# fenghansen/YOND_public

Hardware: AMD Instinct MI355X
Metric: Bayer megapixels/sec end-to-end (NLE+VST+denoise+iVST) (higher is better)
Workload: dtype f32 (3x3 convolutions: f32 operands as two f16 halves -- 22-23 significant bits -- on the f16 MFMA, 3 products per f32 product, f32 accumulate; per-layer error vs float64 asserted <= 2x the f32 direct kernel's and <= 2e-5 of max|ref| (tests/test_hip_conv.py; measured 1.3e-6 vs 1.5e-6), whole frame v

## Files before the change

### include/yond_hip.h

```cpp
#ifndef YOND_HIP_H
#define YOND_HIP_H

#include <stddef.h>
#include <stdint.h>

#ifdef __cplusplus
extern "C" {
#endif

#define YOND_OK 0
#define YOND_EINVAL (-1)
#define YOND_EUNSUPPORTED (-2)

#define YOND_ABI_VERSION 8
int yond_abi_version(void);

int yond_pack_vst_norm_f32(const float* bayer, int H, int W, float* out, int pad_l, int pad_r, int pad_t,
                           int pad_b, int mode, double scale, double gain, double sigma, double lo,
                           double hi, const double* lut_x, const float* lut_y, int lut_n, float* img_max,
                           void* stream);

int yond_pack_vst_norm_biaslut_f32(const float* bayer, int H, int W, float* out, int pad_l, int pad_r, int pad_t,
                                   int pad_b, double scale, double gain, double sigma, double lo, double hi,
                                   const double* lut_x, const double* lut_y, int lut_n, float* img_max, void* stream);
// ... 27 lines not shown

typedef struct YondConvDesc {
    const float* src0;
    const float* src1;
    int C0, C1;
    int N, H, W;
    int Ho, Wo;
    int Cout;
    int ksize;
    int stride;
    int shuffle;
    int pre_act;
    int post_act;
    float slope;
    const float* wpk;
    const float* escale;
    const float* eshift;
    int ebatch;
    const float* res;
    float* dst;
    int tn;
    int kc;
    int algo;
    const float* out4_w;
    const float* out4_b;
    const float* out4_x;
    const float* out4_ub;
    float* out4_dst;
    unsigned int* status;
    int in_fmt, out_fmt;
    int res_fmt;
    unsigned long long* clk;
    int tile_order;
    float* dst2;
} YondConvDesc;
#define YOND_STATUS_HALF_OVERFLOW 1u
#define YOND_FMT_NHWC_F32 0
#define YOND_FMT_SPLIT_PLANES 1
#define YOND_FMT_PLANES4 2
#define YOND_SP_PLANE_UNITS(H, W) ((((H) * (W)) + 8) / 8 * 8)
#define YOND_SP_BYTES(N, C, H, W) ((size_t)(N) * ((C) / 16) * 4 * (size_t)YOND_SP_PLANE_UNITS(H, W) * 16)
#define YOND_HP_BYTES(N, C, H, W) ((size_t)(N) * ((C) / 16) * 2 * (size_t)YOND_SP_PLANE_UNITS(H, W) * 16)

int yond_conv_config(int ksize, int stride, int cin, int cout, int shuffle, int N, int Ho, int Wo, int* tn, int* kc);
int yond_pack_conv_weight_f32(const float* w, int cout, int cin, int ksize, int tn, int kc, float* dst);
int yond_pack_conv_weight_split_f32(const float* w, int cout, int cin, int ksize, int tn, int kc, float* dst);
int yond_conv2d_f32(const YondConvDesc* desc, void* stream);

int yond_conv_wino_supported(int cin, int cout);
int yond_pack_conv_wino_weight_f32(const float* w, int cout, int cin, int tn, float* dst);

int yond_conv_split_supported(int ksize, int stride, int cin, int cout);
int yond_pack_conv_split_weight_f32(const float* w, int cout, int cin, int ksize, int tn, int parts, float* dst);
int yond_pack_conv_split_weight_dev_f32(const float* w, int cout, int cin, int ksize, int tn, int parts, float* dst, int* status,
                                        void* stream);
int yond_pack_conv_split_weights_batch_dev_f32(const float* src, const long long* desc, int nlayers, float* dst, size_t ngroups,
                                               int* status, void* stream);

int yond_conv_in_f32(const float* x, const float* ub , int N, int H, int W, int Cout,
                     const float* wpk, const float* bias, float slope, float* dst,
                     int out_fmt , void* stream);
int yond_pack_conv_in_weight_f32(const float* w , int cout, float* dst );

int yond_conv_out_f32(const float* feat , int Cin, const float* w ,
                      const float* bias , const float* x ,
                      const float* ub , int N, int H, int W, float* dst ,
                      void* stream);

int yond_maxpool2_f32(const float* src, int N, int H, int W, int C, float* dst, void* stream);

typedef struct YondFilmDesc {
    int kind, C, ld;
    const float *w_a0, *b_a0, *w_a2, *b_a2;
    const float *w_b0, *b_b0;
    const float *w_b, *b_b;
    const float *cb1, *cb2;
    float *s1, *t1, *s2, *t2;
} YondFilmDesc;
int yond_film_f32(const YondFilmDesc* descs, int nblocks, const float* t , const float* ub ,
                  int N, void* stream);

int yond_box_stats_self1_f32(const float* bayer, int H, int W, int k, int k2, int tile_w, float* mean,
                             float* var, float* blur2, void* stream);
int yond_box_stats_self2_f32(const float* blur2, int h, int w, int k, int tile_w, float* lap, void* stream);
int yond_box_stats_collab_f32(const float* bayer_lr, const float* bayer_hr, int H, int W, int k, int tile_w,
                              float* mean, float* var, float* lap, void* stream);


int yond_box_stats_self_stats_f32(const float* bayer, int H, int W, int k, int k2, int tile_w, float* mean, float* var,
                                  float* blur2, float* lap, const double* q_host, int nq, void* ws, void* stream);
int yond_box_stats_collab_stats_f32(const float* bayer_lr, const float* bayer_hr, int H, int W, int k, int tile_w,
                                    float* mean, float* var, float* lap, const double* q_host, int nq, void* ws, void* stream);

size_t yond_select_ws_bytes(int nr);
int yond_select_ranks_f32(const float* data, size_t n, const int64_t* ranks_host, int nr, float* out, void* ws,
                          void* stream);
int yond_percentiles_f32(const float* data, size_t n, const double* q_host, int nq, double* out, void* ws,
                         void* stream);

size_t yond_nle_ws_bytes(size_t n);
int yond_nle_stats_f32(const float* lap, const float* mean, size_t n, int width, const double* q_host, int nq, void* ws,
                       void* stream);
int yond_nle_threshold_f32(const float* lap, size_t n, const double* q_host, int nq, int want_score, void* ws, void* stream);
int yond_nle_state_layout(int* off );
int yond_nle_moments_f32(const float* lap, const float* mean, const float* var, size_t n, void* ws, void* stream);

// ... 214 lines not shown
```

### yond_public_amd/_lib.py

```python
import ctypes as C
import os

import torch

_HERE = os.path.dirname(os.path.abspath(__file__))
LIB_PATH = os.environ.get("YOND_HIP_LIB", os.path.join(_HERE, "libyond_hip.so"))
_lib = None
ABI_VERSION = 8

vp, i32, f32, f64, sz, i64 = C.c_void_p, C.c_int, C.c_float, C.c_double, C.c_size_t, C.c_longlong


class YondConvDesc(C.Structure):
    _fields_ = [("src0", vp), ("src1", vp), ("C0", i32), ("C1", i32), ("N", i32), ("H", i32), ("W", i32),
                ("Ho", i32), ("Wo", i32), ("Cout", i32), ("ksize", i32), ("stride", i32), ("shuffle", i32),
                ("pre_act", i32), ("post_act", i32), ("slope", f32), ("wpk", vp), ("escale", vp),
                ("eshift", vp), ("ebatch", i32), ("res", vp), ("dst", vp), ("tn", i32), ("kc", i32), ("algo", i32),
                ("out4_w", vp), ("out4_b", vp), ("out4_x", vp), ("out4_ub", vp), ("out4_dst", vp), ("status", vp),
                ("in_fmt", i32), ("out_fmt", i32), ("res_fmt", i32), ("clk", vp), ("tile_order", i32), ("dst2", vp)]


class YondBlock0Desc(C.Structure):
    _fields_ = [("x", vp), ("in_fmt", i32), ("N", i32), ("H", i32), ("W", i32), ("w1", vp), ("w2", vp),
                ("s1", vp), ("t1", vp), ("s2", vp), ("t2", vp), ("ebatch", i32), ("dst", vp),
                ("out4_w", vp), ("out4_b", vp), ("out4_x", vp), ("out4_ub", vp), ("out4_dst", vp), ("status", vp)]


class YondFilmDesc(C.Structure):
    _fields_ = [("kind", i32), ("C", i32), ("ld", i32),
                ("w_a0", vp), ("b_a0", vp), ("w_a2", vp), ("b_a2", vp), ("w_b0", vp), ("b_b0", vp),
                ("w_b", vp), ("b_b", vp), ("cb1", vp), ("cb2", vp),
                ("s1", vp), ("t1", vp), ("s2", vp), ("t2", vp)]


PROTOTYPES = {
    "yond_abi_version": [],
    "yond_pack_vst_norm_f32": [vp, i32, i32, vp, i32, i32, i32, i32, i32, f64, f64, f64, f64, f64, vp, vp, i32, vp, vp],
    "yond_pack_vst_norm_biaslut_f32": [vp, i32, i32, vp, i32, i32, i32, i32, f64, f64, f64, f64, f64, vp, vp, i32, vp, vp],
    "yond_bias_eval_f32": [vp, sz, vp, vp, i32, i32, i32, f64, f64, vp, vp],
    "yond_denorm_ivst_unpack_f32": [vp, i32, i32, i32, i32, i32, i32, vp, i32, f64, f64, f64, f64, f64, i32, vp],
    "yond_pack_vst_norm_batch_f32": [vp, i32, i32, i32, vp, i32, i32, i32, i32, f64, f64, f64, f64, f64, vp, vp, i32, i32, vp, vp],
    "yond_denorm_ivst_unpack_batch_f32": [vp, i32, i32, i32, i32, i32, i32, i32, vp, i32, f64, f64, f64, f64, f64, i32, vp],
    "yond_vst_elem_f32": [vp, sz, f64, f64, f64, vp, vp],
    "yond_ivst_elem_f64": [vp, sz, f64, f64, i32, vp, vp],
    "yond_bayer2rggb_f32": [vp, i32, i32, vp, vp],
    "yond_rggb2bayer_f32": [vp, i32, i32, vp, vp],
    "yond_rot90_f32": [vp, i32, i32, i32, i32, vp, vp],
    "yond_nchw4_to_nhwc4_f32": [vp, vp, i32, i32, i32, vp],
    "yond_nhwc4_to_nchw4_f32": [vp, vp, i32, i32, i32, vp],
    "yond_image_max_f32": [vp, i32, sz, vp, vp, vp],
    "yond_conv_config": [i32, i32, i32, i32, i32, i32, i32, i32, C.POINTER(i32), C.POINTER(i32)],
    "yond_pack_conv_weight_f32": [vp, i32, i32, i32, i32, i32, vp],
    "yond_conv2d_f32": [C.POINTER(YondConvDesc), vp],
    "yond_conv_wino_supported": [i32, i32],
    "yond_pack_conv_wino_weight_f32": [vp, i32, i32, i32, vp],
    "yond_pack_conv_weight_split_f32": [vp, i32, i32, i32, i32, i32, vp],
    "yond_conv_split_supported": [i32, i32, i32, i32],
    "yond_pack_conv_split_weight_f32": [vp, i32, i32, i32, i32, i32, vp],
    "yond_pack_conv_split_weight_dev_f32": [vp, i32, i32, i32, i32, i32, vp, vp, vp],
    "yond_pack_conv_split_weights_batch_dev_f32": [vp, vp, i32, vp, sz, vp, vp],
    "yond_conv_in_f32": [vp, vp, i32, i32, i32, i32, vp, vp, f32, vp, i32, vp],
    "yond_pack_conv_in_weight_f32": [vp, i32, vp],
    "yond_conv_out_f32": [vp, i32, vp, vp, vp, vp, i32, i32, i32, vp, vp],
    "yond_maxpool2_f32": [vp, i32, i32, i32, i32, vp, vp],
    "yond_film_f32": [vp, i32, vp, vp, i32, vp],
    "yond_box_stats_self1_f32": [vp, i32, i32, i32, i32, i32, vp, vp, vp, vp],
    "yond_box_stats_self2_f32": [vp, i32, i32, i32, i32, vp, vp],
    "yond_box_stats_collab_f32": [vp, vp, i32, i32, i32, i32, vp, vp, vp, vp],
    "yond_box_stats_self_stats_f32": [vp, i32, i32, i32, i32, i32, vp, vp, vp, vp, vp, i32, vp, vp],
    "yond_box_stats_collab_stats_f32": [vp, vp, i32, i32, i32, i32, vp, vp, vp, vp, i32, vp, vp],
    "yond_select_ws_bytes": [i32],
    "yond_select_ranks_f32": [vp, sz, vp, i32, vp, vp, vp],
    "yond_percentiles_f32": [vp, sz, vp, i32, vp, vp, vp],
    "yond_nle_ws_bytes": [sz],
    "yond_nle_stats_f32": [vp, vp, sz, i32, vp, i32, vp, vp],
    "yond_nle_threshold_f32": [vp, sz, vp, i32, i32, vp, vp],
    "yond_nle_state_layout": [vp],
    "yond_nle_moments_f32": [vp, vp, vp, sz, vp, vp],
    "yond_nlf_occupancy_f32": [vp, vp, sz, i32, vp, i32, vp, vp],
    "yond_nlf_score3_f64": [vp, vp, vp, i32, vp, vp, vp],
    "yond_nlf_moments_f32": [vp, vp, vp, sz, vp, vp, vp],
    "yond_bias_lut_f64": [vp, i32, f64, f64, vp, vp],
    "yond_block_metrics_tiles": [i32, i32],
    "yond_block_metrics_f32": [vp, vp, i32, i32, i32, i32, vp, vp],
    "yond_block_metrics_rgb8": [vp, vp, i32, i32, i32, i32, vp, vp],
    "yond_render_srgb": [vp, i32, i32, i32, i32, i32, C.POINTER(f64), C.POINTER(f64), i32, vp, vp, i32, vp, f64, vp],
    "yond_clock_probe": [f64, vp, vp],
    "yond_img2raw_f32": [vp, sz, i32, i32, i32, vp, vp, i32, i32, i32, vp, vp, vp, vp],
    "yond_pg_noise_f32": [vp, vp, sz, i32, vp, i32, vp],
    "yond_camera_noise_f32": [vp, vp, sz, i32, vp, i32, i32, vp],
    "yond_est_conv_in_f32": [vp, i32, i32, i32, i32, vp, vp, vp, vp],
    "yond_est_head_f32": [vp, i32, i32, i32, i32, vp, vp, i32, i32, i32, vp, vp, vp],
    "yond_est_head_ws_bytes": [i32, i32],
    "yond_conv_wgrad_f32": [vp, vp, i32, i32, i32, i32, i32, i32, i32, i32, i32, vp, vp],
    "yond_conv_wgrad_ws_f32": [vp, vp, i32, i32, i32, i32, i32, i32, i32, i32, i32, vp, vp, sz, vp],
    "yond_conv_wgrad_ws_bytes": [i32, i32, i32, i32, i32, i32, i32, i32, i32],
    "yond_conv_wgrad_split_ws_bytes": [i32, i32, i32, i32, i32],
    "yond_conv_wgrad_split_f32": [vp, vp, i32, i32, i32, i32, i32, vp, i32, vp, sz, vp, vp],
    "yond_colsum_f32": [vp, sz, i32, vp, vp],
    "yond_film_silu_supported": [i32],
    "yond_film_silu_f32": [vp, vp, vp, vp, i32, sz, i32, vp],
    "yond_film_silu_bwd_f32": [vp, vp, vp, vp, vp, vp, vp, i32, sz, i32, vp],
    "yond_film_mlp_fwd_f32": [vp, vp, vp, vp, vp, vp, vp, i32, i32, i32, vp, vp, vp],
    "yond_film_mlp_bwd_f32": [vp, vp, vp, vp, vp, vp, vp, vp, i32, i32, i32, vp, vp, vp, vp, vp, vp, vp, vp],
    "yond_film_mlp_fwd_multi_f32": [vp, i32, vp],
    "yond_gemm_split_f32": [vp, i32, sz, i32, i32, i64, i64, i32, vp, vp, i32, i32, i32, i32, vp, vp],
    "yond_film_mlp_bwd_multi_f32": [vp, i32, vp],
    "yond_silu_bwd_add_f32": [vp, vp, vp, vp, sz, vp],
    "yond_silu_f32": [vp, vp, sz, vp],
    "yond_zero_interleave_f32": [vp, i32, i32, i32, i32, i32, i32, vp, vp],
    "yond_l1_loss_f32": [vp, vp, sz, vp, vp, vp],
# ... 113 lines not shown
```

### yond_public_amd/csrc/conv.hip

```cpp
#include "common.h"
#include <cstdlib>

#ifndef YOND_B32_WGS
#define YOND_B32_WGS 2
#endif
#ifndef YOND_ABL
#define YOND_ABL 0
#endif

template <int KS, int STRIDE, int TH, int TN, int KC>
struct ConvCfg {
    static constexpr int TW = 32;
    static constexpr int TAPS = KS * KS;
    static constexpr int PADK = KS / 2;
    static constexpr int IH = (TH - 1) * STRIDE + KS;
    static constexpr int IW = (TW - 1) * STRIDE + KS;
    static constexpr int HALF = (IW + 1) / 2;
    static constexpr int TWP = (STRIDE == 2) ? 2 * HALF : IW;
    static constexpr int PS = KC + 4;
    static constexpr int IN_FLOATS = IH * TWP * PS;
    static constexpr int Q = KC / 8;
    static constexpr int W_FLOATS = TAPS * Q * 2 * TN * 4;
    static constexpr int BUF_FLOATS = IN_FLOATS + W_FLOATS;
    static constexpr int NW = TN / 32;
// ... 466 lines not shown
#ifdef YOND_EXPERIMENTS
    {
        const long e11 = yond_exp_long("YOND_1X1_TN", 0), es2 = yond_exp_long("YOND_S2_TN", 0), ekc = yond_exp_long("YOND_CONV_KC", 0),
                   etn = yond_exp_long("YOND_CONV_TN", 0);
        if (e11 && ksize == 1) t = e11 == 32 ? 32 : (ntile % 64 == 0 ? 64 : 32);
        if (es2 && ksize == 3 && stride == 2) t = es2 == 32 ? 32 : (ntile % 64 == 0 ? 64 : 32);
        if (ekc && ksize == 3 && stride == 1) k = ekc == 8 ? 8 : 16;
        if (etn && ksize == 3 && stride == 1 && ntile % 64 == 0) t = etn == 32 ? 32 : 64;
    }
#endif
    if (tn) *tn = t;
    if (kc) *kc = k;
    return YOND_OK;
}

extern "C" int yond_pack_conv_weight_f32(const float* w, int cout, int cin, int ksize, int tn, int kc, float* dst) {
    if (!w || !dst || (tn != 32 && tn != 64) || cout % tn != 0 || cin % kc != 0 || kc % 8 != 0) return YOND_EINVAL;
    const int taps = ksize * ksize, Q = kc / 8;
    size_t o = 0;
    for (int ct = 0; ct < cout / tn; ++ct)
        for (int ch = 0; ch < cin / kc; ++ch)
            for (int tap = 0; tap < taps; ++tap)
                for (int q = 0; q < Q; ++q)
                    for (int h = 0; h < 2; ++h)
                        for (int j = 0; j < tn; ++j)
                            for (int e = 0; e < 4; ++e) {
                                const int co = ct * tn + j, ci = ch * kc + q * 8 + h * 4 + e;
                                dst[o++] = w[((size_t)co * cin + ci) * taps + tap];
                            }
    return YOND_OK;
}

extern "C" int yond_pack_conv_weight_split_f32(const float* w, int cout, int cin, int ksize, int tn, int kc, float* dst) {
    const int rc = yond_pack_conv_weight_f32(w, cout, cin, ksize, tn, kc, dst);
    if (rc != YOND_OK) return rc;
    const size_t n = (size_t)cout * cin * ksize * ksize;
    for (size_t i = 0; i < n; ++i)
        if (!(fabsf(w[i]) <= 65504.0f)) return YOND_EUNSUPPORTED;
    for (size_t i = 0; i < n; ++i) {
        const float v = dst[i];
        const _Float16 h = (_Float16)v;
        const _Float16 l = (_Float16)((v - (float)h) * 2048.0f);
        unsigned short hb, lb;
        __builtin_memcpy(&hb, &h, 2);
        __builtin_memcpy(&lb, &l, 2);
        const unsigned u = (unsigned)hb | ((unsigned)lb << 16);
        __builtin_memcpy(&dst[i], &u, 4);
    }
    return YOND_OK;
}

int yond_conv_wino_dispatch(const YondConvDesc& d, hipStream_t st);
int yond_conv_split_dispatch(const YondConvDesc& d, hipStream_t st);

extern "C" int yond_conv2d_f32(const YondConvDesc* dp, void* stream) {
    if (!dp) return YOND_EINVAL;
    const YondConvDesc& d = *dp;
    hipStream_t st = (hipStream_t)stream;
    if (!d.src0 || !(d.dst || d.out4_dst) || !d.wpk || d.N <= 0 || d.H <= 0 || d.W <= 0 || d.Ho <= 0 || d.Wo <= 0) return YOND_EINVAL;
    if (d.out4_dst && ((d.algo != 3 && d.algo != 4) || !d.out4_w || d.Cout != 32 || d.stride != 1)) return YOND_EUNSUPPORTED;
    if (d.C1 > 0 && !d.src1) return YOND_EINVAL;
    if (d.shuffle < 0 || d.shuffle > 2) return YOND_EINVAL;
    if (d.shuffle == 2 && d.algo != 3 && d.algo != 4) return YOND_EUNSUPPORTED;
    if ((long long)d.N * d.H * d.W > 0x7fffffffLL) return YOND_EUNSUPPORTED;
    if (d.pre_act != 0 && d.pre_act != 1) return YOND_EINVAL;
    if (d.in_fmt < 0 || d.in_fmt > 2 || d.out_fmt < 0 || d.out_fmt > 2 || (d.res_fmt != 0 && d.res_fmt != 2)) return YOND_EINVAL;
    if ((d.in_fmt || d.out_fmt || d.res_fmt) && d.algo != 3 && d.algo != 4) return YOND_EUNSUPPORTED;
    if (d.algo == 1) return yond_conv_wino_dispatch(d, st);
    if (d.algo == 3 || d.algo == 4) return yond_conv_split_dispatch(d, st);
    if (d.algo != 0 && d.algo != 2 && d.algo != 5) return YOND_EINVAL;
    if (d.tn != 32 && d.tn != 64) return YOND_EINVAL;
    int tn, kc;
    const int rc = yond_conv_config(d.ksize, d.stride, d.C0 + d.C1, d.Cout, d.shuffle, 0, 0, 0, &tn, &kc);
    if (rc != YOND_OK) return rc;
    tn = d.tn;
    if (d.kc != 0) kc = d.kc;
    if (kc != 8 && kc != 16) return YOND_EINVAL;
    if (kc == 8 && d.ksize != 3) return YOND_EINVAL;
    if (d.ksize == 3 && d.stride == 2 && kc != 8) return YOND_EINVAL;
    if (d.C0 % kc != 0 || d.C1 % kc != 0 || d.Cout % tn != 0) return YOND_EUNSUPPORTED;
    if (d.shuffle && (d.ksize != 1 || (d.Cout / 4) % tn != 0)) return YOND_EUNSUPPORTED;
    if ((long long)d.N * d.H * d.W > 0x7fffffffLL) return YOND_EUNSUPPORTED;
    if (d.stride == 2) {
        if (d.Ho != (d.H + 1) / 2 || d.Wo != (d.W + 1) / 2) return YOND_EINVAL;
    } else if (d.Ho != d.H || d.Wo != d.W) return YOND_EINVAL;
    if (d.pre_act != 0 && d.pre_act != 1) return YOND_EINVAL;
    if (d.post_act != 0 && d.post_act != 2) return YOND_EUNSUPPORTED;
    if (d.pre_act == 1 && !(d.ksize == 3 && d.stride == 1)) return YOND_EUNSUPPORTED;
    if (d.ksize == 3 && d.stride == 1 && kc == 8) {
        if (d.pre_act) return tn == 64 ? launch_conv<3, 1, 8, 64, 8, true>(d, st) : launch_conv<3, 1, 8, 32, 8, true>(d, st);
        return tn == 64 ? launch_conv<3, 1, 8, 64, 8, false>(d, st) : launch_conv<3, 1, 8, 32, 8, false>(d, st);
    }
    if (d.ksize == 3 && d.stride == 1) {
        if (d.pre_act) return tn == 64 ? launch_conv<3, 1, 8, 64, 16, true>(d, st) : launch_conv<3, 1, 8, 32, 16, true>(d, st);
        return tn == 64 ? launch_conv<3, 1, 8, 64, 16, false>(d, st) : launch_conv<3, 1, 8, 32, 16, false>(d, st);
    }
    if (d.ksize == 3 && d.stride == 2)
        return tn == 64 ? launch_conv<3, 2, 8, 64, 8, false>(d, st) : launch_conv<3, 2, 4, 32, 8, false>(d, st);
    return tn == 64 ? launch_conv<1, 1, 8, 64, 16, false>(d, st) : launch_conv<1, 1, 8, 32, 16, false>(d, st);
}
```

### yond_public_amd/engine.py

```python
import ctypes as C
import os

import numpy as np
import torch

from . import _lib as L


def _rup(c, m=32):
    return (c + m - 1) // m * m


def _np_ptr(a):
    return C.c_void_p(a.ctypes.data)


FILM_MAX_C = 1024


WINO_DEFAULT = 'split'


SPLIT_PLANES = True
SP_FLOW = True
HALF_FLOW = True
HALF_K1_TN128 = True
HALF_S2_TN128 = True
HALF_FLOW_TN128 = True
HALF_TN128 = True
FUSE_OUT4 = True
FUSE_BLOCK0 = False
K1_SUB2 = True
K1_D2_LEVELS = (3,)
K1_D2_LEVELS_HALF = ()
SP_CONV1_MIN_LEVEL = 3
UNET_SP = True
SNAKE_ORDER = True


def sp_plane_units(H, W):
    return (H * W + 8) // 8 * 8


class _PackedConv:

    def __init__(self, dev, weight, bias, ksize, stride, splits, shuffle=False):
        lib = L.load()
        w = weight.detach().to('cpu', torch.float32).numpy()
        if shuffle:
            cin, cout = w.shape[0], w.shape[1]
            coutp = _rup(cout)
            m = np.zeros((4, coutp, cin), np.float32)
            m[:, :cout, :] = w.transpose(2, 3, 1, 0).reshape(4, cout, cin)
            w = m.reshape(4 * coutp, cin, 1, 1)
            self.cout_real_p = coutp
            gemm_n = 4 * coutp
        else:
            cout = w.shape[0]
            coutp = _rup(cout)
            gemm_n = coutp
            self.cout_real_p = coutp
        assert sum(splits) == w.shape[1], (splits, w.shape)
        psplits = [_rup(s) for s in splits]
        cinp = sum(psplits)
        wp = np.zeros((gemm_n, cinp, ksize, ksize), np.float32)
        so, do = 0, 0
        for s, ps in zip(splits, psplits):
            wp[:w.shape[0], do:do + s] = w[:, so:so + s]
            so += s
            do += ps
        self._wp = np.ascontiguousarray(wp)
        self._packed = {}
        self._dev = dev
        b = torch.zeros(coutp, dtype=torch.float32)
        if bias is not None:
            b[:cout] = bias.detach().to('cpu', torch.float32)
        self.bias = b.to(dev)
        self.ksize, self.stride, self.shuffle = ksize, stride, shuffle
        self.psplits, self.gemm_n, self.coutp, self.cinp = psplits, gemm_n, coutp, cinp
        self.cin_real, self.cout_real = sum(splits), cout
        self.config(0, 0, 0)
        self.wmax = float(np.abs(self._wp).max()) if self._wp.size else 0.0
        self.macs_per_pixel = self.cin_real * self.cout_real * (4 if shuffle else ksize * ksize)

    def config(self, N, Ho, Wo, split=False):
        lib = L.load()
# ... 174 lines not shown
            raise L.YondHipError(f"first layer must have 4 input channels (packed Bayer), got {w.shape[1]}")
        coutp = _rup(cout)
        wp = np.zeros((coutp, 4, 3, 3), np.float32)
        wp[:cout] = w
        packed = np.empty(coutp * 40, np.float32)
        L.check(self.lib.yond_pack_conv_in_weight_f32(_np_ptr(wp), coutp, _np_ptr(packed)), "yond_pack_conv_in_weight_f32")
        bp = torch.zeros(coutp, dtype=torch.float32)
        bp[:cout] = b.detach().to('cpu', torch.float32)
        return torch.from_numpy(packed).to(self.dev), bp.to(self.dev)

    def _pad_out_w(self, w):
        w = w.detach().to('cpu', torch.float32).reshape(w.shape[0], -1)
        if w.shape[0] != 4:
            raise L.YondHipError(f"last layer must have 4 output channels, got {w.shape[0]}")
        wp = torch.zeros(4, _rup(w.shape[1]), dtype=torch.float32)
        wp[:, :w.shape[1]] = w
        return wp.to(self.dev).contiguous()

    def _split_pair(self, pc1, pc2):
        if getattr(self, 'strict', False) or getattr(self, 'conv_algo', WINO_DEFAULT) != 'split':
            return False
        prec = getattr(self, 'precision', 'fp32')
        if prec not in ('fp32', 'fp16'):
            return False
        parts = 2 if prec == 'fp32' else 1
        return all(pc.ksize == 3 and pc.stride == 1 and pc.split(parts) is not None for pc in (pc1, pc2))

    def _sp_flow(self, N, H, W):
        if not (SPLIT_PLANES and SP_FLOW) or getattr(self, 'strict', False) or getattr(self, 'conv_algo', WINO_DEFAULT) != 'split':
            return False
        prec = getattr(self, 'precision', 'fp32')
        if prec not in ('fp32', 'fp16') or (prec == 'fp16' and not HALF_FLOW) or sp_plane_units(H, W) * 64 * 4 >= 2 ** 31:
            return False
        parts = 2 if prec == 'fp32' else 1
        for i, blk in self.blocks.items():
            for k in ('conv1', 'conv2', 'pool', 'upsc'):
                if k in blk and blk[k].split(parts, wide=False) is None:
                    return False
        return self._out4_fusable(self.blocks[9]['conv2'], flow=True)

    def _out4_fusable(self, pc, flow=False):
        prec = getattr(self, 'precision', 'fp32')
        return (not getattr(self, 'strict', False) and getattr(self, 'conv_algo', WINO_DEFAULT) == 'split' and (prec == 'fp32' or (prec == 'fp16' and flow))
                and pc.ksize == 3 and pc.stride == 1 and pc.gemm_n == 32 and pc.split(2 if prec == 'fp32' else 1) is not None and FUSE_OUT4)

    def _new_sp(self, key, N, H, W, Cc, parts=2):
        cache = self.__dict__.setdefault('_sp_cache', {})
        k = (key, N, H, W, Cc, parts, getattr(self, 'lane', 0))
        if k not in cache:
            cache[k] = torch.zeros(N * (Cc // 16) * 2 * parts * sp_plane_units(H, W) * 4, dtype=torch.float32, device=self.dev)
        return cache[k]

    def _conv(self, pc, src0, src1, N, H, W, dst, escale=None, eshift=None, ebatch=0, res=None, pre_act=0, post_act=0,
              slope=0.0, algo=None, out4=None, in_fmt=0, out_fmt=0, res_fmt=0, dst2=None):
        d = L.YondConvDesc()
        d.src0 = src0.data_ptr()
        d.src1 = src1.data_ptr() if src1 is not None else None
        d.C0 = pc.psplits[0]
        d.C1 = pc.psplits[1] if len(pc.psplits) > 1 else 0
        d.N, d.H, d.W = N, H, W
        if pc.stride == 2:
            d.Ho, d.Wo = (H + 1) // 2, (W + 1) // 2
        else:
            d.Ho, d.Wo = H, W
        d.Cout = pc.gemm_n
        d.ksize, d.stride, d.shuffle = pc.ksize, pc.stride, int(pc.shuffle)
        d.pre_act, d.post_act, d.slope = pre_act, post_act, slope
        prec = getattr(self, 'precision', 'fp32')
        if getattr(self, 'strict', False) and algo is None:
            prec, algo = 'fp32-mfma', 1
        if algo is None:
            algo = getattr(self, 'conv_algo', WINO_DEFAULT)
            if prec == 'fp32-mfma' and algo == 'split':
                algo = 1
            if prec == 'fp16' and WINO_DEFAULT == 'split':
                algo = 'half'
        fp16 = prec == 'fp16' or algo == 'fp16'
        wino = split = None
        if algo in ('split', 'half'):
            ws2 = (HALF_S2_TN128 and algo == 'half' and pc.stride == 2 and in_fmt == 1 and out_fmt == 2 and dst2 is None
                   and (pc.gemm_n // 128) * ((d.Wo + 31) // 32) * ((d.Ho + 7) // 8) * N >= 256)
            ws2 = ws2 or (HALF_K1_TN128 and algo == 'half' and pc.ksize == 1 and in_fmt == 1 and dst2 is None)
            split = pc.split(2 if algo == 'split' else 1, wide=(not (in_fmt or out_fmt or res_fmt or dst2 is not None)) or (HALF_FLOW_TN128 and out_fmt == 1),
                             wide_s2=ws2)
            if algo == 'half' and pc.ksize == 1 and in_fmt != 1:
                split = None
            if split is None and not fp16 and pc.ksize == 3:
                wino = pc.wino()
        elif not fp16:
            wino = pc.wino() if algo in (1, 2) else None
        if split is not None:
            tn, wpk = split
            kc = 16
            d.algo = 3 if algo == 'split' else 4
        elif wino is not None:
            tn, wpk = wino
            kc = 8
            d.algo = 1
        elif algo == 'split' and pc.ksize == 1 and not fp16 and pc.config(N, d.Ho, d.Wo, split=True)[2] is not None:
            tn, kc, wpk = pc.config(N, d.Ho, d.Wo, split=True)
            d.algo = 5
        else:
            tn, kc, wpk = pc.config(N, d.Ho, d.Wo)
            d.algo = 2 if (fp16 and pc.wmax <= 65504.0) else 0
        d.wpk = wpk.data_ptr()
        d.tn = tn
        d.kc = kc
        d.escale = escale.data_ptr() if escale is not None else None
        d.eshift = (eshift if eshift is not None else pc.bias).data_ptr()
        d.ebatch = ebatch
        d.res = res.data_ptr() if res is not None else None
        d.dst = dst.data_ptr() if dst is not None else None
        status = getattr(self, 'status', None)
        d.status = status.data_ptr() + 4 * self.status_slot if status is not None else None
        d.in_fmt, d.out_fmt, d.res_fmt = in_fmt, out_fmt, res_fmt
        d.dst2 = dst2.data_ptr() if dst2 is not None else None
        if SNAKE_ORDER and d.algo in (3, 4):
            self._tile_order = 1 - getattr(self, '_tile_order', 0)
            d.tile_order = self._tile_order
        clk = getattr(self, 'clk', None)
        d.clk = clk.data_ptr() if (clk is not None and d.algo in (3, 4)) else None
        if (in_fmt or out_fmt or res_fmt) and d.algo not in (3, 4):
            raise L.YondHipError("split-plane / 4-channel-plane tensors need the split-operand kernel (algo 3, or 4 with h-only planes)")
        if out4 is not None:
            w4, b4, x4, ub4, o4 = out4
            if d.algo not in (3, 4):
                raise L.YondHipError("fused output projection needs the split-operand 3x3 kernel")
            d.out4_w, d.out4_b = w4.data_ptr(), (b4.data_ptr() if b4 is not None else None)
            d.out4_x = x4.data_ptr() if x4 is not None else None
            d.out4_ub = ub4.data_ptr() if ub4 is not None else None
            d.out4_dst = o4.data_ptr()
        prof = getattr(self, 'prof', None)
        if prof is not None:
            tag = f"conv_wino_kernel<{tn}>" if d.algo == 1 else f"conv_mfma_kernel<{pc.ksize},{pc.stride},8,{tn},{kc}>"
            if d.algo in (3, 4):
                tag = f"conv_split_kernel<{pc.stride if pc.ksize == 3 else 'k1'},{tn},{5 - d.algo}>"
            if d.algo == 2:
                tag += "/f16"
            if d.algo == 5:
                tag += "/split"
            only = getattr(self, 'prof_only', None)
            if only is not None and not only(tag):
                prof = None
            every = getattr(self, 'prof_every', 1)
            if every > 1 and getattr(self, '_fwd_idx', 0) % every:
                prof = None
        if prof is not None:
            e0, e1 = torch.cuda.Event(enable_timing=True), torch.cuda.Event(enable_timing=True)
            e0.record()
        L.check(self.lib.yond_conv2d_f32(C.byref(d), L.stream()), "yond_conv2d_f32")
        if prof is not None:
            e1.record()
            prof.append((tag, 2.0 * pc.macs_per_pixel * N * d.Ho * d.Wo, e0, e1))
        return dst

    def _block0_weights(self, pc):
        w = getattr(pc, '_b0', None)
        if w is None:
            if not L.has("yond_pack_block0_weight_f32"):
                raise L.YondHipError("the fused level-0 block exists only in experiment builds of the library (python -m yond_public_amd.build --experiments)")
            if not (pc.ksize == 3 and pc.stride == 1 and pc.gemm_n == 32 and pc.cinp == 32 and len(pc.psplits) == 1):
                return None
            host = np.zeros(9 * 2 * 4 * 32 * 8, np.float16)
            if self.lib.yond_pack_block0_weight_f32(_np_ptr(pc._wp), 32, 32, _np_ptr(host)) != 0:
                return None
            w = pc._b0 = torch.from_numpy(host.view(np.float32)).to(pc._dev)
        return w

    def _block0(self, pc1, pc2, x, N, H, W, f, in_fmt, dst=None, out4=None):
        w1, w2 = self._block0_weights(pc1), self._block0_weights(pc2)
        d = L.YondBlock0Desc()
        d.x, d.in_fmt, d.N, d.H, d.W = x.data_ptr(), in_fmt, N, H, W
        d.w1, d.w2 = w1.data_ptr(), w2.data_ptr()
        d.s1, d.t1, d.s2, d.t2 = (None if v is None else v.data_ptr() for v in f)
        d.ebatch = 1
        d.dst = dst.data_ptr() if dst is not None else None
        if out4 is not None:
            w4, b4, x4, ub4, o4 = out4
            d.out4_w, d.out4_b = w4.data_ptr(), (b4.data_ptr() if b4 is not None else None)
            d.out4_x = x4.data_ptr() if x4 is not None else None
            d.out4_ub = ub4.data_ptr() if ub4 is not None else None
            d.out4_dst = o4.data_ptr()
        status = getattr(self, 'status', None)
        d.status = status.data_ptr() + 4 * self.status_slot if status is not None else None
        prof = getattr(self, 'prof', None)
        if prof is not None:
            tag = "block0_fused_kernel" + ("<o4>" if out4 is not None else "")
            only = getattr(self, 'prof_only', None)
            if (only is not None and not only(tag)) or (getattr(self, 'prof_every', 1) > 1 and getattr(self, '_fwd_idx', 0) % getattr(self, 'prof_every', 1)):
# ... 51 lines not shown

    def overflowed(self, slot=0):
        return bool(int(self.status[slot].item()) & 1)

    def image_max(self, x4, N):
        elems = x4.numel() // N
        partial = torch.empty(N * 256, dtype=torch.float32, device=self.dev)
        ub = torch.empty(N, dtype=torch.float32, device=self.dev)
        L.check(self.lib.yond_image_max_f32(L.ptr(x4), N, elems, L.ptr(partial), L.ptr(ub), L.stream()), "yond_image_max_f32")
        return ub

    def _new(self, N, H, W, Cc):
        return torch.empty((N, H, W, Cc), dtype=torch.float32, device=self.dev)

    def forward_nhwc4(self, x4, t_dev=None, ub=None):
        L.require_cuda(x4, "x")
        self._fwd_idx = getattr(self, '_fwd_idx', -1) + 1
        self._tile_order = 0
        N, H, W, c4 = x4.shape
        if c4 != 4 or H % 16 or W % 16:
            raise L.YondHipError(f"input must be [N][H][W][4] with H, W multiples of 16, got {tuple(x4.shape)}")
        if self.norm and ub is None:
            ub = self.image_max(x4, N)
        if not self.norm:
            ub = None
        st = L.stream()
        lib = self.lib
        nfp = _rup(self.nf)
        if self.guided:
            if t_dev is None:
                raise L.YondHipError(f"{self.kind}.forward needs the noise level t")
            film = self._film(t_dev, ub, N)
            flow = self._sp_flow(N, H, W)
            pt = 1 if (flow and getattr(self, 'precision', 'fp32') == 'fp16') else 2
            P4, SP = 2, 1
            a = self._new(N, H, W, nfp)
            L.check(lib.yond_conv_in_f32(L.ptr(x4), L.ptr(ub), N, H, W, nfp, L.ptr(self.conv_in_w), L.ptr(self.conv_in_b),
                                         0.01, L.ptr(a), P4 if flow else 0, st), "yond_conv_in_f32")
            skips = {}
            h, w = H, W
            cur = a
            xsp = None
            for i in range(1, 10):
                blk = self.blocks[i]
                cp = blk['Cp']
                f = film[f'conv{i}']
                last = i == 9
                xfmt = P4 if (flow and not last) else 0
                if i >= 6:
                    xs = self._new(N, 2 * h, 2 * w, cp)
                    up = blk['upsc2'] if (flow and K1_SUB2 and 'upsc2' in blk) else blk['upsc']
                    xsp = (self._new_sp(('xspd', i), N, 2 * h, 2 * w, cp, pt)
                           if (flow and not last and (9 - i) in (K1_D2_LEVELS if pt == 2 else K1_D2_LEVELS_HALF) and up is blk['upsc'] and cp % 64 == 0 and w > 16) else None)
                    self._conv(up, cur, skips[10 - i], N, h, w, xs, in_fmt=SP if flow else 0, out_fmt=xfmt, dst2=xsp)
                    h, w = 2 * h, 2 * w
                    cur = xs
                if flow and FUSE_BLOCK0 and h == H and cp == 32 and self._block0_weights(blk['conv1']) is not None and self._block0_weights(blk['conv2']) is not None:
                    if last and self._out4_fusable(blk['conv2'], flow):
                        out4 = self._new(N, H, W, 4)
                        self._block0(blk['conv1'], blk['conv2'], cur, N, h, w, f, xfmt, out4=(self.w_out, self.b_out, x4 if self.res else None, ub, out4))
                        return out4
                    if not last:
                        out = self._new_sp(('out', i), N, h, w, cp, pt)
                        self._block0(blk['conv1'], blk['conv2'], cur, N, h, w, f, xfmt, dst=out)
                        cur = out
                        skips[i] = cur
                        nxt = self._new(N, h // 2, w // 2, blk['pool'].coutp)
                        xsp = self._new_sp(('xsp', i + 1), N, h // 2, w // 2, blk['pool'].coutp, pt) if (flow and i >= SP_CONV1_MIN_LEVEL) else None
                        self._conv(blk['pool'], cur, None, N, h, w, nxt, in_fmt=SP, out_fmt=P4, dst2=xsp)
                        h, w = h // 2, w // 2
                        cur = nxt
                        continue
                act_in_producer = self._split_pair(blk['conv1'], blk['conv2'])
                sp = SP if (flow or (act_in_producer and SPLIT_PLANES and getattr(self, 'precision', 'fp32') == 'fp32'
                                      and sp_plane_units(h, w) * 64 < 2 ** 31)) else 0
                tmp = self._new_sp(('tmp', i), N, h, w, cp, pt) if sp else self._new(N, h, w, cp)
                if xsp is not None and sp and act_in_producer:
                    self._conv(blk['conv1'], xsp, None, N, h, w, tmp, escale=f[0], eshift=f[1], ebatch=1, pre_act=0, post_act=1,
                               in_fmt=SP, out_fmt=sp)
                else:
                    self._conv(blk['conv1'], cur, None, N, h, w, tmp, escale=f[0], eshift=f[1], ebatch=1, pre_act=1,
                               post_act=1 if act_in_producer else 0, in_fmt=xfmt, out_fmt=sp)
                xsp = None
                pre2 = 0 if act_in_producer else 1
                if last and self._out4_fusable(blk['conv2'], flow):
                    out4 = self._new(N, H, W, 4)
                    self._conv(blk['conv2'], tmp, None, N, h, w, None, escale=f[2], eshift=f[3], ebatch=1, res=cur, pre_act=pre2,
                               out4=(self.w_out, self.b_out, x4 if self.res else None, ub, out4), in_fmt=sp)
                    return out4
                if flow:
                    out = self._new_sp(('out', i), N, h, w, cp, pt)
                    self._conv(blk['conv2'], tmp, None, N, h, w, out, escale=f[2], eshift=f[3], ebatch=1, res=cur, pre_act=pre2,
                               in_fmt=SP, out_fmt=SP, res_fmt=P4)
                else:
                    out = self._new(N, h, w, cp)
                    self._conv(blk['conv2'], tmp, None, N, h, w, out, escale=f[2], eshift=f[3], ebatch=1, res=cur, pre_act=pre2, in_fmt=sp)
                cur = out
                if i <= 4:
                    skips[i] = cur
                    nxt = self._new(N, h // 2, w // 2, blk['pool'].coutp)
                    xsp = self._new_sp(('xsp', i + 1), N, h // 2, w // 2, blk['pool'].coutp, pt) if (flow and i >= SP_CONV1_MIN_LEVEL) else None
                    self._conv(blk['pool'], cur, None, N, h, w, nxt, in_fmt=SP if flow else 0, out_fmt=P4 if flow else 0, dst2=xsp)
                    h, w = h // 2, w // 2
                    cur = nxt
            feat = cur
        else:
            a = self._new(N, H, W, nfp)
# ... 76 lines not shown
```

Measured before the change: 2576.

## Add weight-stationary persistent 1x1 upsample GEMM kernel for decoder levels

Adds a new persistent kernel (algo 6) for the 1x1 upsample convolutions at the three shallowest decoder levels. Each workgroup holds its 64-output-channel weight slice and FiLM scale/shift in LDS, and each wave streams 32-pixel segments through a register ring of prefetched split-f16 input chunks, issuing the split-precision MFMAs with a fused FiLM/leaky epilogue and pixel-shuffle store. The aim is to avoid reloading weights per tile and to overlap global loads with MFMA work. It adds a fixed 256-block grid and large LDS use, which may limit occupancy or balance on small frames.

```diff
diff --git a/include/yond_hip.h b/include/yond_hip.h
--- a/include/yond_hip.h
+++ b/include/yond_hip.h
@@ -103,6 +103,7 @@
 
 int yond_conv_split_supported(int ksize, int stride, int cin, int cout);
 int yond_pack_conv_split_weight_f32(const float* w, int cout, int cin, int ksize, int tn, int parts, float* dst);
+int yond_gemm_k1_stationary_supported(const YondConvDesc* desc);
 int yond_pack_conv_split_weight_dev_f32(const float* w, int cout, int cin, int ksize, int tn, int parts, float* dst, int* status,
                                         void* stream);
 int yond_pack_conv_split_weights_batch_dev_f32(const float* src, const long long* desc, int nlayers, float* dst, size_t ngroups,
diff --git a/yond_public_amd/_lib.py b/yond_public_amd/_lib.py
--- a/yond_public_amd/_lib.py
+++ b/yond_public_amd/_lib.py
@@ -57,6 +57,7 @@
     "yond_pack_conv_weight_split_f32": [vp, i32, i32, i32, i32, i32, vp],
     "yond_conv_split_supported": [i32, i32, i32, i32],
     "yond_pack_conv_split_weight_f32": [vp, i32, i32, i32, i32, i32, vp],
+    "yond_gemm_k1_stationary_supported": [C.POINTER(YondConvDesc)],
     "yond_pack_conv_split_weight_dev_f32": [vp, i32, i32, i32, i32, i32, vp, vp, vp],
     "yond_pack_conv_split_weights_batch_dev_f32": [vp, vp, i32, vp, sz, vp, vp],
     "yond_conv_in_f32": [vp, vp, i32, i32, i32, i32, vp, vp, f32, vp, i32, vp],
diff --git a/yond_public_amd/csrc/conv.hip b/yond_public_amd/csrc/conv.hip
--- a/yond_public_amd/csrc/conv.hip
+++ b/yond_public_amd/csrc/conv.hip
@@ -542,6 +542,7 @@
 
 int yond_conv_wino_dispatch(const YondConvDesc& d, hipStream_t st);
 int yond_conv_split_dispatch(const YondConvDesc& d, hipStream_t st);
+int yond_gemm_k1_stationary_dispatch(const YondConvDesc& d, hipStream_t st);
 
 extern "C" int yond_conv2d_f32(const YondConvDesc* dp, void* stream) {
     if (!dp) return YOND_EINVAL;
@@ -551,10 +552,11 @@
     if (d.out4_dst && ((d.algo != 3 && d.algo != 4) || !d.out4_w || d.Cout != 32 || d.stride != 1)) return YOND_EUNSUPPORTED;
     if (d.C1 > 0 && !d.src1) return YOND_EINVAL;
     if (d.shuffle < 0 || d.shuffle > 2) return YOND_EINVAL;
-    if (d.shuffle == 2 && d.algo != 3 && d.algo != 4) return YOND_EUNSUPPORTED;
+    if (d.shuffle == 2 && d.algo != 3 && d.algo != 4 && d.algo != 6) return YOND_EUNSUPPORTED;
     if ((long long)d.N * d.H * d.W > 0x7fffffffLL) return YOND_EUNSUPPORTED;
     if (d.pre_act != 0 && d.pre_act != 1) return YOND_EINVAL;
     if (d.in_fmt < 0 || d.in_fmt > 2 || d.out_fmt < 0 || d.out_fmt > 2 || (d.res_fmt != 0 && d.res_fmt != 2)) return YOND_EINVAL;
+    if (d.algo == 6) return yond_gemm_k1_stationary_dispatch(d, st);
     if ((d.in_fmt || d.out_fmt || d.res_fmt) && d.algo != 3 && d.algo != 4) return YOND_EUNSUPPORTED;
     if (d.algo == 1) return yond_conv_wino_dispatch(d, st);
     if (d.algo == 3 || d.algo == 4) return yond_conv_split_dispatch(d, st);
diff --git a/yond_public_amd/csrc/gemm_k1_stationary.hip b/yond_public_amd/csrc/gemm_k1_stationary.hip
--- /dev/null
+++ b/yond_public_amd/csrc/gemm_k1_stationary.hip
@@ -0,0 +1,245 @@
+#include "common.h"
+
+typedef _Float16 f16x8 __attribute__((ext_vector_type(8)));
+typedef unsigned u32x4 __attribute__((ext_vector_type(4)));
+
+template <int NCH, int NLO, int D, bool S2 = false>
+__global__ __launch_bounds__(512) void gemm_k1_stationary_kernel(const YondConvDesc d) {
+    constexpr int WS = NCH % 2 == 0 ? 2 : 3;
+    static_assert(NCH % D == 0 && NCH % WS == 0 && D >= 2 && NLO > 0 && NLO < NCH, "the ring holds whole rounds of a segment's chunks");
+    constexpr int NHI = NCH - NLO;
+    constexpr int CRC = S2 ? NHI / 2 : NHI;
+    constexpr int FILM_OFF = NCH * 1024, EP_OFF = FILM_OFF + 16 * 128, EPS = 36;
+    extern __shared__ __attribute__((aligned(16))) float smem[];
+    const int tid = threadIdx.x, lane = tid & 63, wave = __builtin_amdgcn_readfirstlane(tid >> 6);
+    const int li = lane & 31, lh = lane >> 5;
+    const int Cr = d.Cout / 4, nct = d.Cout / 64;
+    const int per_xcd = gridDim.x / 8;
+    const int bx = blockIdx.x % 8, bj = blockIdx.x / 8;
+    const int ct = bj % nct, grp = bx * (per_xcd / nct) + bj / nct, ngrp = gridDim.x / nct;
+    const bool clk_on = d.clk != nullptr && blockIdx.x == 0 && tid == 0;
+    unsigned long long clk_c0 = 0, clk_r0 = 0;
+    if (clk_on) { clk_c0 = __builtin_amdgcn_s_memtime(); clk_r0 = __builtin_amdgcn_s_memrealtime(); }
+
+    {
+        const f32x4* wsrc = (const f32x4*)(d.wpk + (size_t)ct * NCH * 1024);
+        f32x4* wl = (f32x4*)smem;
+        for (int i = tid; i < NCH * 256; i += 512) wl[i] = wsrc[i];
+        float* film = smem + FILM_OFF;
+        const int nfilm = d.ebatch ? d.N : 1;
+        for (int i = tid; i < nfilm * 128; i += 512) {
+            const int im = i >> 7, k = i & 127;
+            const int cb = (ct * 64 + (k & 63)) % Cr;
+            film[i] = k < 64 ? (d.escale ? d.escale[im * Cr + cb] : 1.0f) : (d.eshift ? d.eshift[im * Cr + cb] : 0.0f);
+        }
+    }
+    __syncthreads();
+
+    const int nsx = (d.W + 31) / 32;
+    const long long nseg = (long long)d.N * d.H * nsx;
+    const long long sstep = 8LL * ngrp;
+    const long long s0 = grp + (long long)ngrp * wave;
+    if (s0 < nseg) {
+        const bool rev = d.tile_order != 0;
+        const size_t PS0 = (size_t)YOND_SP_PLANE_UNITS(d.H, d.W) * 16, PS1 = (size_t)YOND_SP_PLANE_UNITS(2 * d.H, 2 * d.W) * 16;
+        const int sp = S2 ? 2 * ct : (ct * 64) / Cr, cb0 = S2 ? 0 : (ct * 64) % Cr;
+        const int Hout = 2 * d.H, Wout = 2 * d.W;
+        const float slope_eff = d.post_act == 2 ? d.slope : 1.0f;
+        struct Geo { int n, y, x; unsigned vlo, vhi, vhi1; };
+        auto geo = [&](long long s) {
+            Geo g;
+            const long long t = rev ? nseg - 1 - s : s;
+            const int per = d.H * nsx;
+            g.n = (int)(t / per);
+            const int r = (int)(t - (long long)g.n * per);
+            g.y = r / nsx;
+            g.x = (r - g.y * nsx) * 32 + li;
+            const bool in = g.x < d.W;
+            g.vlo = (unsigned)((size_t)lh * 2 * PS0) + (unsigned)(in ? g.y * d.W + g.x : d.H * d.W) * 16u;
+            g.vhi = (unsigned)((size_t)lh * 2 * PS1) + (unsigned)(in ? (2 * g.y + (sp >> 1)) * Wout + 2 * g.x + (sp & 1) : Hout * Wout) * 16u;
+            g.vhi1 = in ? g.vhi + 16u : g.vhi;
+            return g;
+        };
+        f16x8 ring[D][2];
+        auto issue = [&](auto cc, const Geo& g) __attribute__((always_inline)) {
+            constexpr int c = decltype(cc)::value, slot = c % D;
+            if constexpr (c < NLO) {
+                const char* b = (const char*)d.src0 + ((size_t)g.n * NLO + c) * 4 * PS0;
+                ring[slot][0] = *(const f16x8*)(b + g.vlo);
+                ring[slot][1] = *(const f16x8*)(b + PS0 + g.vlo);
+            } else {
+                constexpr int k = c - NLO, q = S2 ? k / CRC : 0;
+                constexpr int ch = q < 2 ? k - q * CRC : 0;
+                const char* b = (const char*)d.src1 + ((size_t)g.n * CRC + ch) * 4 * PS1;
+                const unsigned v = q == 1 ? g.vhi1 : g.vhi;
+                ring[slot][0] = *(const f16x8*)(b + v);
+                ring[slot][1] = *(const f16x8*)(b + PS1 + v);
+            }
+        };
+        typedef const __attribute__((address_space(3))) f16x8* lds_h8;
+        const __attribute__((address_space(3))) float* wb = (const __attribute__((address_space(3))) float*)(smem + (lh * 2 * 64 + li) * 4);
+        const float* film = smem + FILM_OFF;
+        const unsigned hw_out = (unsigned)(Hout * Wout);
+        const __amdgpu_buffer_rsrc_t orsrc = __builtin_amdgcn_make_buffer_rsrc(d.dst, 0, (int)((unsigned)d.N * (unsigned)Cr * hw_out * 4u), 0x00020000);
+        f16x8 wt[WS][2][2];
+        auto load_w = [&](auto cc) __attribute__((always_inline)) {
+            constexpr int c = decltype(cc)::value;
+#pragma unroll
+            for (int nn = 0; nn < 2; ++nn)
+#pragma unroll
+                for (int p = 0; p < 2; ++p) wt[c % WS][nn][p] = *(lds_h8)(wb + ((c * 4 + p) * 64 + nn * 32) * 4);
+        };
+
+        auto segment = [&](const Geo& cur, const Geo& nxt) __attribute__((always_inline)) {
+            f32x16 acc[2][2];
+#pragma unroll
+            for (int a = 0; a < 2; ++a)
+#pragma unroll
+                for (int nn = 0; nn < 2; ++nn)
+#pragma unroll
+                    for (int r = 0; r < 16; ++r) acc[a][nn][r] = 0.0f;
+            static_for<0, NCH>([&](auto cc) __attribute__((always_inline)) {
+                constexpr int c = decltype(cc)::value, slot = c % D, ws = c % WS;
+                load_w(IntC<(c + 1) % NCH>{});
+                const f16x8 xh = ring[slot][0], xl = ring[slot][1];
+#pragma unroll
+                for (int nn = 0; nn < 2; ++nn) acc[1][nn] = __builtin_amdgcn_mfma_f32_32x32x16_f16(wt[ws][nn][0], xl, acc[1][nn], 0, 0, 0);
+#pragma unroll
+                for (int nn = 0; nn < 2; ++nn) acc[0][nn] = __builtin_amdgcn_mfma_f32_32x32x16_f16(wt[ws][nn][0], xh, acc[0][nn], 0, 0, 0);
+#pragma unroll
+                for (int nn = 0; nn < 2; ++nn) acc[1][nn] = __builtin_amdgcn_mfma_f32_32x32x16_f16(wt[ws][nn][1], xh, acc[1][nn], 0, 0, 0);
+                if constexpr (c + D < NCH) issue(IntC<c + D>{}, cur);
+                else issue(IntC<c + D - NCH>{}, nxt);
+                __builtin_amdgcn_sched_barrier(0);
+            });
+            if constexpr (S2) {
+                float* sw = smem + EP_OFF + wave * (32 * EPS);
+                const int pj = lane >> 3, u = lane & 7;
+                const int x0 = cur.x - li;
+                const unsigned rowb = (unsigned)((cur.n * Hout + 2 * cur.y + (sp >> 1)) * Wout + 2 * x0);
+                const float* fv = film + (d.ebatch ? cur.n * 128 : 0) + 4 * u;
+#pragma unroll
+                for (int nn = 0; nn < 2; ++nn) {
+#pragma unroll
+                    for (int g = 0; g < 4; ++g) {
+                        f32x4 v;
+#pragma unroll
+                        for (int e = 0; e < 4; ++e) v[e] = fmaf(acc[1][nn][4 * g + e], 1.0f / 2048.0f, acc[0][nn][4 * g + e]);
+                        *(f32x4*)(sw + li * EPS + 8 * g + 4 * lh) = v;
+                    }
+                    const f32x4 es = *(const f32x4*)(fv + nn * 32), et = *(const f32x4*)(fv + 64 + nn * 32);
+#pragma unroll
+                    for (int j = 0; j < 4; ++j) {
+                        const int pp = pj + 8 * j;
+                        const f32x4 x = *(const f32x4*)(sw + pp * EPS + 4 * u);
+                        f32x4 v;
+#pragma unroll
+                        for (int e = 0; e < 4; ++e) {
+                            float y = fmaf(x[e], es[e], et[e]);
+                            y = y > 0.0f ? y : y * slope_eff;
+                            v[e] = y + 0.0f;
+                        }
+                        const unsigned off = (((rowb + 2u * (unsigned)pp + (unsigned)nn) * 32u + 4u * (unsigned)u) * 4u) | (x0 + pp < d.W ? 0u : 0x80000000u);
+                        __builtin_amdgcn_raw_buffer_store_b128(__builtin_bit_cast(u32x4, v), orsrc, (int)off, 0, 0);
+                    }
+                }
+                return;
+            }
+            const unsigned pixo = (unsigned)((2 * cur.y + (sp >> 1)) * Wout + 2 * cur.x + (sp & 1));
+            const unsigned mask = cur.x < d.W ? 0u : 0x80000000u;
+            const float* fv = film + (d.ebatch ? cur.n * 128 : 0) + 4 * lh;
+#pragma unroll
+            for (int nn = 0; nn < 2; ++nn) {
+                const int cbase = cb0 + nn * 32 + 4 * lh;
+                const unsigned ob = (((unsigned)(cur.n * (Cr / 4) + cbase / 4) * hw_out + pixo) * 16u) | mask;
+#pragma unroll
+                for (int g = 0; g < 4; ++g) {
+                    const f32x4 es = *(const f32x4*)(fv + nn * 32 + 8 * g), et = *(const f32x4*)(fv + 64 + nn * 32 + 8 * g);
+                    f32x4 v;
+#pragma unroll
+                    for (int e = 0; e < 4; ++e) {
+                        float x = acc[0][nn][4 * g + e];
+                        x = fmaf(acc[1][nn][4 * g + e], 1.0f / 2048.0f, x);
+                        x = fmaf(x, es[e], et[e]);
+                        x = x > 0.0f ? x : x * slope_eff;
+                        v[e] = x + 0.0f;
+                    }
+                    __builtin_amdgcn_raw_buffer_store_b128(__builtin_bit_cast(u32x4, v), orsrc, (int)(ob + (unsigned)g * 32u * hw_out), 0, 0);
+                }
+            }
+        };
+
+        Geo cur = geo(s0);
+        static_for<0, D>([&](auto cc) { issue(cc, cur); });
+        load_w(IntC<0>{});
+        long long sn = s0 + sstep;
+        Geo nxt = sn < nseg ? geo(sn) : cur;
+        segment(cur, nxt);
+        while (sn < nseg) {
+            cur = nxt;
+            sn += sstep;
+            nxt = sn < nseg ? geo(sn) : cur;
+            segment(cur, nxt);
+        }
+        asm volatile("s_waitcnt vmcnt(0)" ::: "memory");
+    }
+    if (clk_on) {
+        atomicAdd(d.clk, __builtin_amdgcn_s_memtime() - clk_c0);
+        atomicAdd(d.clk + 1, __builtin_amdgcn_s_memrealtime() - clk_r0);
+    }
+}
+
+static int k1s_chunks(const YondConvDesc& d) {
+    if (d.ksize != 1 || d.stride != 1 || (d.shuffle != 1 && d.shuffle != 2) || d.tn != 64 || !d.src0 || !d.src1 || !d.dst || !d.wpk) return 0;
+    if (d.in_fmt != YOND_FMT_SPLIT_PLANES || d.res_fmt || d.res || d.dst2 || d.out4_dst || d.pre_act) return 0;
+    if (d.out_fmt != (d.shuffle == 2 ? YOND_FMT_NHWC_F32 : YOND_FMT_PLANES4)) return 0;
+    if (d.post_act != 0 && d.post_act != 2) return 0;
+    if (d.Ho != d.H || d.Wo != d.W || d.N <= 0 || d.H <= 0 || d.W <= 0 || d.Cout <= 0 || d.Cout % 128) return 0;
+    const int Cr = d.Cout / 4, nct = d.Cout / 64;
+    if (d.shuffle == 2) {
+        if (Cr != 32 || d.C0 != 64 || d.C1 != 80) return 0;
+    } else if (d.Cout % 256 || 32 % nct || d.C0 != 2 * Cr || d.C1 != Cr) return 0;
+    if (d.ebatch && d.N > 16) return 0;
+    if ((long long)d.N * d.H * d.W > 0x7fffffffLL) return 0;
+    if ((long long)d.N * Cr * 4 * d.H * d.W * 4 >= 0x7fffffffLL) return 0;
+    if ((long long)YOND_SP_PLANE_UNITS(d.H, d.W) * 4 * 16 * 4 >= 0x7fffffffLL) return 0;
+    const int nch = (d.C0 + d.C1) / 16;
+    if (d.shuffle == 2) return nch == 9 ? nch : 0;
+    return (nch == 24 || nch == 12) ? nch : 0;
+}
+
+extern "C" int yond_gemm_k1_stationary_supported(const YondConvDesc* d) { return (d && (d->algo == 3 || d->algo == 6) && k1s_chunks(*d)) ? 1 : 0; }
+
+template <int NCH, int NLO, int D, bool S2 = false>
+static int launch_k1s(const YondConvDesc& d, hipStream_t st) {
+    constexpr int SMEM = (NCH * 1024 + 16 * 128 + (S2 ? 8 * 32 * 36 : 0)) * 4;
+    static_assert(SMEM <= 160 * 1024, "LDS budget");
+    static bool attr_set = false;
+    auto kern = gemm_k1_stationary_kernel<NCH, NLO, D, S2>;
+    if (!attr_set) {
+        hipError_t e = hipFuncSetAttribute((const void*)kern, hipFuncAttributeMaxDynamicSharedMemorySize, SMEM);
+        if (e != hipSuccess) return (int)e;
+        attr_set = true;
+    }
+    constexpr int K1S_GRID = 256;
+    static_assert(K1S_GRID % 8 == 0, "whole XCD shares");
+    hipLaunchKernelGGL(kern, dim3(K1S_GRID), dim3(512), SMEM, st, d);
+    YOND_LAUNCH_CHECK();
+    return YOND_OK;
+}
+
+int yond_gemm_k1_stationary_dispatch(const YondConvDesc& d, hipStream_t st) {
+    const int nch = k1s_chunks(d);
+#ifdef YOND_EXPERIMENTS
+    const long depth = yond_exp_long("YOND_K1S_DEPTH", 0);
+    if (nch == 24 && depth == 4) return launch_k1s<24, 16, 4>(d, st);
+    if (nch == 24 && depth == 8) return launch_k1s<24, 16, 8>(d, st);
+    if (nch == 12 && depth == 4) return launch_k1s<12, 8, 4>(d, st);
+    if (nch == 12 && depth == 12) return launch_k1s<12, 8, 12>(d, st);
+    if (nch == 9 && depth == 3) return launch_k1s<9, 4, 3, true>(d, st);
+#endif
+    if (nch == 24) return launch_k1s<24, 16, 6>(d, st);
+    if (nch == 12) return launch_k1s<12, 8, 6>(d, st);
+    if (nch == 9) return launch_k1s<9, 4, 9, true>(d, st);
+    return YOND_EUNSUPPORTED;
+}
diff --git a/yond_public_amd/engine.py b/yond_public_amd/engine.py
--- a/yond_public_amd/engine.py
+++ b/yond_public_amd/engine.py
@@ -32,6 +32,7 @@
 FUSE_BLOCK0 = False
 K1_SUB2 = True
 K1_D2_LEVELS = (3,)
+K1_STATIONARY_LEVELS = (2, 1, 0)
 K1_D2_LEVELS_HALF = ()
 SP_CONV1_MIN_LEVEL = 3
 UNET_SP = True
@@ -312,7 +313,7 @@
         return cache[k]
 
     def _conv(self, pc, src0, src1, N, H, W, dst, escale=None, eshift=None, ebatch=0, res=None, pre_act=0, post_act=0,
-              slope=0.0, algo=None, out4=None, in_fmt=0, out_fmt=0, res_fmt=0, dst2=None):
+              slope=0.0, algo=None, out4=None, in_fmt=0, out_fmt=0, res_fmt=0, dst2=None, stationary=False):
         d = L.YondConvDesc()
         d.src0 = src0.data_ptr()
         d.src1 = src1.data_ptr() if src1 is not None else None
@@ -375,12 +376,14 @@
         d.status = status.data_ptr() + 4 * self.status_slot if status is not None else None
         d.in_fmt, d.out_fmt, d.res_fmt = in_fmt, out_fmt, res_fmt
         d.dst2 = dst2.data_ptr() if dst2 is not None else None
-        if SNAKE_ORDER and d.algo in (3, 4):
+        if stationary and d.algo == 3 and self.lib.yond_gemm_k1_stationary_supported(C.byref(d)):
+            d.algo = 6
+        if SNAKE_ORDER and d.algo in (3, 4, 6):
             self._tile_order = 1 - getattr(self, '_tile_order', 0)
             d.tile_order = self._tile_order
         clk = getattr(self, 'clk', None)
-        d.clk = clk.data_ptr() if (clk is not None and d.algo in (3, 4)) else None
-        if (in_fmt or out_fmt or res_fmt) and d.algo not in (3, 4):
+        d.clk = clk.data_ptr() if (clk is not None and d.algo in (3, 4, 6)) else None
+        if (in_fmt or out_fmt or res_fmt) and d.algo not in (3, 4, 6):
             raise L.YondHipError("split-plane / 4-channel-plane tensors need the split-operand kernel (algo 3, or 4 with h-only planes)")
         if out4 is not None:
             w4, b4, x4, ub4, o4 = out4
@@ -393,8 +396,8 @@
         prof = getattr(self, 'prof', None)
         if prof is not None:
             tag = f"conv_wino_kernel<{tn}>" if d.algo == 1 else f"conv_mfma_kernel<{pc.ksize},{pc.stride},8,{tn},{kc}>"
-            if d.algo in (3, 4):
-                tag = f"conv_split_kernel<{pc.stride if pc.ksize == 3 else 'k1'},{tn},{5 - d.algo}>"
+            if d.algo in (3, 4, 6):
+                tag = f"conv_split_kernel<{pc.stride if pc.ksize == 3 else 'k1'},{tn},{1 if d.algo == 4 else 2}>" + ("/stationary" if d.algo == 6 else "")
             if d.algo == 2:
                 tag += "/f16"
             if d.algo == 5:
@@ -552,7 +555,8 @@
                     up = blk['upsc2'] if (flow and K1_SUB2 and 'upsc2' in blk) else blk['upsc']
                     xsp = (self._new_sp(('xspd', i), N, 2 * h, 2 * w, cp, pt)
                            if (flow and not last and (9 - i) in (K1_D2_LEVELS if pt == 2 else K1_D2_LEVELS_HALF) and up is blk['upsc'] and cp % 64 == 0 and w > 16) else None)
-                    self._conv(up, cur, skips[10 - i], N, h, w, xs, in_fmt=SP if flow else 0, out_fmt=xfmt, dst2=xsp)
+                    self._conv(up, cur, skips[10 - i], N, h, w, xs, in_fmt=SP if flow else 0, out_fmt=xfmt, dst2=xsp,
+                               stationary=(9 - i) in K1_STATIONARY_LEVELS)
                     h, w = 2 * h, 2 * w
                     cur = xs
                 if flow and FUSE_BLOCK0 and h == H and cp == 32 and self._block0_weights(blk['conv1']) is not None and self._block0_weights(blk['conv2']) is not None:
```

Result: faster. 2666, median of 6 (+3.5%).
